# AdamBeedell/MLX8-WS-Audio-Transformer

Hardware: AMD Instinct MI355X
Metric: 4s@16kHz clips/sec through mel+Whisper-small encoder (higher is better)
Workload: dtype fp16; 1 GPU; int16 PCM [B,64000] in HBM -> Whisper log-mel [B,80,3000] -> Whisper-small encoder -> hidden [B,1500,768] fp32; mode=parity (clip zero-padded to 30 s, as the reference computes), precision=f16f8, fp16_exact_projection_matrices=0 of 48 (found by the library at upload), parallelism=dp1 (clip shards, no data-path collective)

## Files before the change

mlx8-ws-audio-transformer_amd/csrc/attention_f8.hip:

```cpp
#include <type_traits>
#include "common.h"

extern int g_attn_shape;

namespace {

typedef int i32x4_t __attribute__((ext_vector_type(4)));

constexpr int KB = 64;
constexpr int PL16 = KB * 64 * 2;
constexpr int PL8 = KB * 64;
constexpr int STAGE = 2 * PL16 + 4 * PL8;
constexpr int OFF_K16 = 0, OFF_V16 = PL16, OFF_K8 = 2 * PL16, OFF_KL8 = 2 * PL16 + PL8, OFF_V8 = 2 * PL16 + 2 * PL8, OFF_VL8 = 2 * PL16 + 3 * PL8;

struct Attn8Args {
  const bf16_t *q16, *k16, *v16;
  const uint8_t *q8, *ql8, *k8, *kl8, *v8, *vl8;
  bf16_t* o16; uint8_t *o8, *ol8; float* o_f32;
  float* lse;
  int B, H, S;
  char* o_ilv;
};

__device__ __forceinline__ int swz16(int row) { return (row >> 1) & 7; }
__device__ __forceinline__ int swz_v16(int row) { return ((row >> 1) & 1) << 2; }
__device__ __forceinline__ int swz_k8(int row) { return (row >> 2) & 3; }
__device__ __forceinline__ int swz_v8(int row) { return ((row >> 3) & 1) << 1; }

template <int E>
__device__ __forceinline__ int fp8x4_scaled(float a, float b, float c, float d) {
  typedef short s16x2 __attribute__((ext_vector_type(2)));
  constexpr float inv = pow2f(-E);
  s16x2 r = {0, 0};
  r = __builtin_amdgcn_cvt_scalef32_pk_fp8_f32(r, a, b, inv, false);
  r = __builtin_amdgcn_cvt_scalef32_pk_fp8_f32(r, c, d, inv, true);
  return __builtin_bit_cast(int, r);
}

constexpr int K3_SLOT = PL16 + 2 * PL8, V3_SLOT = PL16, K3_O8 = PL16, K3_OL8 = PL16 + PL8, V3_BASE = 3 * K3_SLOT, RING3_BYTES = 3 * (K3_SLOT + V3_SLOT);
template <int NW>
struct KvLaneOff {
  unsigned o16[8 / NW];
  unsigned o16v[8 / NW];
  unsigned o8k, o8v;
};
template <int NW>
__device__ __forceinline__ KvLaneOff<NW> kv_lane_off(int last, int wave, int lane) {
  KvLaneOff<NW> o;
#pragma unroll
  for (int i = 0; i < 8 / NW; ++i) {
    const int p = (i * NW + wave) * 64 + lane, row = p >> 3;
    o.o16[i] = (unsigned)(min(row, last) * 64 + (((p & 7) ^ swz16(row)) << 3)) * 2u;
    o.o16v[i] = (unsigned)(min(row, last) * 64 + (((p & 7) ^ swz_v16(row)) << 3)) * 2u;
  }
  const int p = (wave & 3) * 64 + lane, row = p >> 2;
  o.o8k = (unsigned)(min(row, last) * 64 + (((p & 3) ^ swz_k8(row)) << 4));
  o.o8v = (unsigned)(min(row, last) * 64 + (((p & 3) ^ swz_v8(row)) << 4));
  return o;
}
template <int NW, bool ISK, bool W8 = true, bool RING3 = false>
__device__ __forceinline__ void stage_kv1(const Attn8Args& a, int64_t head_off, int kt, unsigned stage, int wave, const KvLaneOff<NW>& lo) {
  const int64_t tile_off = head_off + (int64_t)kt * (KB * 64);
  const bf16_t* p16 = (ISK ? a.k16 : a.v16) + tile_off;
  const uint8_t* p8 = (ISK ? a.k8 : a.v8) + tile_off;
  const uint8_t* pl8 = (ISK ? a.kl8 : a.vl8) + tile_off;
  constexpr int O16 = RING3 ? 0 : (ISK ? OFF_K16 : OFF_V16), O8 = RING3 ? K3_O8 : (ISK ? OFF_K8 : OFF_V8), OL8 = RING3 ? K3_OL8 : (ISK ? OFF_KL8 : OFF_VL8);
#pragma unroll
  for (int i = 0; i < 8 / NW; ++i) glds16_asm_sbase(p16, ISK ? lo.o16[i] : lo.o16v[i], stage + O16 + (i * NW + wave) * 1024);
  if constexpr (!W8) return;
  const int grp = wave & 3;
  const unsigned off = ISK ? lo.o8k : lo.o8v;
  if (NW == 4) {
    glds16_asm_sbase(p8, off, stage + O8 + grp * 1024);
    glds16_asm_sbase(pl8, off, stage + OL8 + grp * 1024);
  } else {
    glds16_asm_sbase(wave < 4 ? p8 : pl8, off, stage + (wave < 4 ? O8 : OL8) + grp * 1024);
  }
}

template <int NW, bool PV8>
__global__ __launch_bounds__(64 * NW, 2) void attention_f16f8_pipe_kernel(Attn8Args a) {
  constexpr int QB = 32 * NW;
  extern __shared__ __attribute__((aligned(16))) char smem[];
  const int lane = threadIdx.x & 63;
  const int wave = __builtin_amdgcn_readfirstlane(threadIdx.x >> 6);
  const int nqb = (a.S + QB - 1) / QB;
  const int nwg = nqb * a.B * a.H;
  const int logical = xcd_contiguous(blockIdx.x, nwg);
  const int bh = logical / nqb;
  const int b = bh / a.H, h = bh - b * a.H;
  const int q0 = (logical - bh * nqb) * QB + wave * 32;
  const int64_t head_off = (int64_t)bh * a.S * 64;
  const int ql = lane & 31, half = lane >> 5;

  bf16x8 q16[4];
  i32x8 q8, ql8;
  {
    int q = q0 + ql; q = q < a.S ? q : a.S - 1;
    const int64_t off = head_off + (int64_t)q * 64;
#pragma unroll
    for (int ks = 0; ks < 4; ++ks) q16[ks] = *reinterpret_cast<const bf16x8*>(a.q16 + off + half * 8 + ks * 16);
    const uint4 x0 = *reinterpret_cast<const uint4*>(a.q8 + off + half * 32), x1 = *reinterpret_cast<const uint4*>(a.q8 + off + half * 32 + 16);
    const uint4 y0 = *reinterpret_cast<const uint4*>(a.ql8 + off + half * 32), y1 = *reinterpret_cast<const uint4*>(a.ql8 + off + half * 32 + 16);
    q8 = (i32x8){(int)x0.x, (int)x0.y, (int)x0.z, (int)x0.w, (int)x1.x, (int)x1.y, (int)x1.z, (int)x1.w};
    ql8 = (i32x8){(int)y0.x, (int)y0.y, (int)y0.z, (int)y0.w, (int)y1.x, (int)y1.y, (int)y1.z, (int)y1.w};
  }
  f32x16 oacc[2] = {(f32x16){}, (f32x16){}};
  float m_run = -1.0e30f, l_run = 0.f;

  int koff[4], k8off[2];
#pragma unroll
  for (int ks = 0; ks < 4; ++ks) koff[ks] = ql * 128 + (((2 * ks + half) ^ swz16(ql)) << 4);
#pragma unroll
  for (int c = 0; c < 2; ++c) k8off[c] = ql * 64 + (((2 * half + c) ^ swz_k8(ql)) << 4);
  const int g = lane >> 4, li = lane & 15, qq = li >> 2, pp = li & 3;
  const int vkey = 4 * (g >> 1) + qq;
  const int voff = vkey * 128 + (((2 * (g & 1) + (pp >> 1)) ^ swz_v16(vkey)) << 4) + 8 * (pp & 1);
  const int voffx = voff ^ 64;
  const int tq = li >> 1, tp = li & 1;
  const int v8key = 8 * (tq >> 2) + (tq & 3) + 4 * (g >> 1);
  const int v8off = v8key * 64 + ((((g & 1)) ^ swz_v8(v8key)) << 4) + 8 * tp;

  const int ntiles = (a.S + KB - 1) / KB;

  constexpr int NSLOT = PV8 ? 24 : 20, DEPTH = 2, RING = DEPTH + 1;
  constexpr bool RING3 = !PV8;
  static_assert(!RING3 || NW == 4, "the ring form runs on four waves (its counted vmcnt waits assume one group of each e4m3 plane per wave)");
  constexpr int KO8 = RING3 ? K3_O8 : OFF_K8, KOL8 = RING3 ? K3_OL8 : OFF_KL8, VO16 = RING3 ? 0 : OFF_V16;
  const unsigned lds0 = (unsigned)(uintptr_t)(__attribute__((address_space(3))) const char*)(smem);
  auto kslot = [&](int t) -> unsigned { return RING3 ? lds0 + (t % 3) * K3_SLOT : lds0 + (t & 1) * STAGE; };
  auto vslot = [&](int t) -> unsigned { return RING3 ? lds0 + V3_BASE + (t % 3) * V3_SLOT : lds0 + (t & 1) * STAGE; };
  struct RdAddr { unsigned k16[4], k8[2], v0, v1, v8[2]; };
  auto rd_addr = [&](unsigned kb, unsigned vb) {
    RdAddr r;
    constexpr bool PIN = !PV8;
#pragma unroll
    for (int ks = 0; ks < 4; ++ks) { r.k16[ks] = kb + koff[ks]; if constexpr (PIN) asm volatile("" : "+v"(r.k16[ks])); }
#pragma unroll
    for (int c = 0; c < 2; ++c) { r.k8[c] = kb + k8off[c]; if constexpr (PIN) asm volatile("" : "+v"(r.k8[c])); }
    r.v0 = vb + VO16 + voff; r.v1 = vb + VO16 + voffx;
    if constexpr (PIN) asm volatile("" : "+v"(r.v0), "+v"(r.v1));
    if constexpr (PV8) { r.v8[0] = vb + v8off; r.v8[1] = vb + (v8off ^ 32); }
    else r.v8[0] = r.v8[1] = 0;
    return r;
  };
  auto lds128 = [](unsigned addr) { return *(const __attribute__((address_space(3))) i32x4_t*)(uintptr_t)addr; };
  auto read_slot = [&](auto slot_t, const RdAddr& ra, i32x8& f) {
    constexpr int SLOT = decltype(slot_t)::value;
    if constexpr (SLOT < 12) {
      constexpr int kt2 = SLOT / 6, w = SLOT % 6;
      if constexpr (w < 2) {
        constexpr int pl = (w == 0 ? KO8 : KOL8) + kt2 * 2048;
        const i32x4_t x0 = lds128(ra.k8[0] + pl), x1 = lds128(ra.k8[1] + pl);
        f = (i32x8){x0[0], x0[1], x0[2], x0[3], x1[0], x1[1], x1[2], x1[3]};
      } else {
        const i32x4_t x0 = lds128(ra.k16[w - 2] + kt2 * 4096);
        f[0] = x0[0]; f[1] = x0[1]; f[2] = x0[2]; f[3] = x0[3];
      }
    } else if constexpr (SLOT < 20) {
      constexpr int I = SLOT - 12, kt2 = I >> 2, s2 = (I >> 1) & 1, et = I & 1;
      constexpr int cst = kt2 * 4096 + s2 * 2048;
      const unsigned a0 = (et == 0 ? ra.v0 : ra.v1) + cst, a1 = a0 + 1024;
      const i32x2 va = __builtin_bit_cast(i32x2, __builtin_amdgcn_ds_read_tr16_b64_v4i16((__attribute__((address_space(3))) bf16x4*)(uintptr_t)a0));
      const i32x2 vb2 = __builtin_bit_cast(i32x2, __builtin_amdgcn_ds_read_tr16_b64_v4i16((__attribute__((address_space(3))) bf16x4*)(uintptr_t)a1));
      f[0] = va[0]; f[1] = va[1]; f[2] = vb2[0]; f[3] = vb2[1];
    } else {
      constexpr int I = SLOT - 20, et = I >> 1, lo = I & 1;
#pragma unroll
      for (int n = 0; n < 4; ++n) {
        const i32x2 x = __builtin_amdgcn_ds_read_tr8_b64_v2i32((__attribute__((address_space(3))) i32x2*)(uintptr_t)(ra.v8[et] + (lo ? OFF_VL8 : OFF_V8) + n * 1024));
        f[2 * n] = x[0]; f[2 * n + 1] = x[1];
      }
    }
  };
  const KvLaneOff<NW> lo_full = kv_lane_off<NW>(KB - 1, wave, lane);
  auto lane_off = [&](int t) -> KvLaneOff<NW> {
    if ((a.S % KB) != 0 && t == ntiles - 1) return kv_lane_off<NW>(a.S - 1 - t * KB, wave, lane);
    return lo_full;
  };

  stage_kv1<NW, true, true, RING3>(a, head_off, 0, kslot(0), wave, lane_off(0));
  stage_kv1<NW, false, PV8, RING3>(a, head_off, 0, vslot(0), wave, lane_off(0));
  if (ntiles > 1) stage_kv1<NW, true, true, RING3>(a, head_off, 1, kslot(1), wave, lane_off(1));
  if constexpr (RING3) {
    if (ntiles > 1) stage_kv1<NW, false, PV8, RING3>(a, head_off, 1, vslot(1), wave, lane_off(1));
    if (ntiles > 2) stage_kv1<NW, true, true, RING3>(a, head_off, 2, kslot(2), wave, lane_off(2));
  }
  asm volatile("s_waitcnt vmcnt(0)" ::: "memory");
  __syncthreads();
  f32x16 sa[2], sb[2];
  auto qk_mma = [&](auto slot_t, const i32x8& f, f32x16 (&sn)[2]) {
    constexpr int SLOT = decltype(slot_t)::value, kt2 = SLOT / 6, w = SLOT % 6;
    if constexpr (w == 0) sn[kt2] = mfma32_f8<e8m0(-kF8KV), e8m0(-kF8Q - kF8Lo)>(f, ql8, (f32x16){});
    else if constexpr (w == 1) sn[kt2] = mfma32_f8<e8m0(-kF8KV - kF8Lo), e8m0(-kF8Q)>(f, q8, sn[kt2]);
    else {
      const bf16x8 kh = __builtin_bit_cast(bf16x8, (i32x4_t){f[0], f[1], f[2], f[3]});
      sn[kt2] = mfma32<true>(kh, q16[w - 2], sn[kt2]);
    }
  };
  {
    i32x8 ring[RING];
    const RdAddr ra0 = rd_addr(kslot(0), vslot(0));
    [&]<int... P>(std::integer_sequence<int, P...>) { (read_slot(std::integral_constant<int, P>{}, ra0, ring[P]), ...); }(std::make_integer_sequence<int, DEPTH>{});
    [&]<int... I>(std::integer_sequence<int, I...>) {
      ([&] {
        if constexpr (I + DEPTH < 12) read_slot(std::integral_constant<int, I + DEPTH>{}, ra0, ring[(I + DEPTH) % RING]);
        qk_mma(std::integral_constant<int, I>{}, ring[I % RING], sa);
      }(), ...);
    }(std::make_integer_sequence<int, 12>{});
  }
  asm volatile("s_waitcnt lgkmcnt(0)" ::: "memory");
  __syncthreads();

  auto iter = [&](auto last_t, auto tail_t, int kt, f32x16 (&sc)[2], f32x16 (&sn)[2]) {
    constexpr bool LAST = decltype(last_t)::value, TAIL = decltype(tail_t)::value;
    constexpr int FIRST = LAST ? 12 : 0;
    const RdAddr ra = rd_addr(kslot(kt + 1), vslot(kt));
    if constexpr (!LAST) {
      if constexpr (RING3) {
        if (kt + 3 < ntiles) stage_kv1<NW, true, true, true>(a, head_off, kt + 3, kslot(kt), wave, lane_off(kt + 3));
        if (kt + 2 < ntiles) stage_kv1<NW, false, false, true>(a, head_off, kt + 2, vslot(kt + 2), wave, lane_off(kt + 2));
      } else {
        if (kt + 2 < ntiles) stage_kv1<NW, true>(a, head_off, kt + 2, kslot(kt), wave, lane_off(kt + 2));
        stage_kv1<NW, false, PV8>(a, head_off, kt + 1, vslot(kt + 1), wave, lane_off(kt + 1));
      }
    }
    bf16x8 p16[4];
    i32x8 p8, pl8;
    float tmax = -1.0e30f, m_new, alpha, psum = 0.f;
    auto valu_chunk = [&](auto c_t) {
      constexpr int C = decltype(c_t)::value;
      if constexpr (C < 2) {
#pragma unroll
        for (int r = 0; r < 16; ++r) {
          if (TAIL) {
            const int key = kt * KB + C * 32 + (r & 3) + 8 * (r >> 2) + 4 * half;
            sc[C][r] = key < a.S ? sc[C][r] : -1.0e30f;
          }
          tmax = fmaxf(tmax, sc[C][r]);
        }
        if constexpr (C == 1) {
          tmax = fmaxf(tmax, __shfl_xor(tmax, 32));
          m_new = fmaxf(m_run, tmax);
          alpha = __builtin_amdgcn_exp2f(m_run - m_new);
          m_run = m_new;
        }
      } else if constexpr (C < 10) {
        constexpr int e = C - 2, kt2 = e >> 2, r4 = e & 3;
#pragma unroll
        for (int j = 0; j < 4; ++j) {
          const float pv = __builtin_amdgcn_exp2f(sc[kt2][4 * r4 + j] - m_new);
          sc[kt2][4 * r4 + j] = pv;
          psum += pv;
          p16[2 * kt2 + (r4 >> 1)][4 * (r4 & 1) + j] = (short)f32_to_f16(pv);
        }
      } else if constexpr (C < 12) {
        constexpr int et = C - 10;
#pragma unroll
        for (int r = 0; r < 16; ++r) {
          oacc[et][r] *= alpha;
        }
        if constexpr (et == 1) l_run = l_run * alpha + psum;
      } else if constexpr (C < 20 && PV8) {
        constexpr int I = C - 12, c2 = I >> 2, r4 = I & 3;
        float lo[4];
#pragma unroll
        for (int j = 0; j < 4; ++j) lo[j] = __builtin_fmaf(f16_to_f32((bf16_t)p16[2 * c2 + (r4 >> 1)][4 * (r4 & 1) + j]), -1.0f, sc[c2][4 * r4 + j]);
        p8[4 * c2 + r4] = fp8x4_scaled<kF8P>(sc[c2][4 * r4], sc[c2][4 * r4 + 1], sc[c2][4 * r4 + 2], sc[c2][4 * r4 + 3]);
        pl8[4 * c2 + r4] = fp8x4_scaled<kF8P + kF8Lo>(lo[0], lo[1], lo[2], lo[3]);
      }
    };
    auto mma = [&](auto slot_t, const i32x8& f) {
      constexpr int SLOT = decltype(slot_t)::value;
      if constexpr (SLOT < 12) qk_mma(slot_t, f, sn);
      else if constexpr (SLOT < 20) {
        constexpr int I = SLOT - 12, kt2 = I >> 2, s2 = (I >> 1) & 1, et = I & 1;
        const bf16x8 vh = __builtin_bit_cast(bf16x8, (i32x4_t){f[0], f[1], f[2], f[3]});
        oacc[et] = mfma32<true>(vh, p16[2 * kt2 + s2], oacc[et]);
      } else {
        constexpr int I = SLOT - 20, et = I >> 1, lo = I & 1;
        if constexpr (lo == 0) oacc[et] = mfma32_f8<e8m0(-kF8KV), e8m0(-kF8P - kF8Lo)>(f, pl8, oacc[et]);
        else oacc[et] = mfma32_f8<e8m0(-kF8KV - kF8Lo), e8m0(-kF8P)>(f, p8, oacc[et]);
      }
    };
    i32x8 ring[RING];
    [&]<int... P>(std::integer_sequence<int, P...>) { (read_slot(std::integral_constant<int, FIRST + P>{}, ra, ring[(FIRST + P) % RING]), ...); }(std::make_integer_sequence<int, DEPTH>{});
    if constexpr (LAST) {
      [&]<int... C>(std::integer_sequence<int, C...>) { (valu_chunk(std::integral_constant<int, C>{}), ...); }(std::make_integer_sequence<int, 12>{});
    }
    [&]<int... J>(std::integer_sequence<int, J...>) {
      ([&] {
        constexpr int I = FIRST + J;
        if constexpr (I + DEPTH < NSLOT) read_slot(std::integral_constant<int, I + DEPTH>{}, ra, ring[(I + DEPTH) % RING]);
        if constexpr (!LAST || I >= 12) valu_chunk(std::integral_constant<int, I>{});
        __builtin_amdgcn_sched_barrier(0);
        mma(std::integral_constant<int, I>{}, ring[I % RING]);
        __builtin_amdgcn_sched_barrier(0);
      }(), ...);
    }(std::make_integer_sequence<int, NSLOT - FIRST>{});
    if constexpr (RING3 && !LAST) {
      constexpr int NK = 8 / NW + 2, NV = 8 / NW;
      if (kt + 3 < ntiles) asm volatile("s_waitcnt vmcnt(%0)" ::"n"(NK + NV) : "memory");
      else if (kt + 2 < ntiles) asm volatile("s_waitcnt vmcnt(%0)" ::"n"(NV) : "memory");
      else asm volatile("s_waitcnt vmcnt(0)" ::: "memory");
    } else {
      asm volatile("s_waitcnt vmcnt(0)" ::: "memory");
    }
    __syncthreads();
  };
  int kt = 0;
  for (; kt + 2 < ntiles; kt += 2) {
    iter(std::false_type{}, std::false_type{}, kt, sa, sb);
    iter(std::false_type{}, std::false_type{}, kt + 1, sb, sa);
  }
  if (kt + 2 == ntiles) {
    iter(std::false_type{}, std::false_type{}, kt, sa, sb);
    if (a.S % KB) iter(std::true_type{}, std::true_type{}, kt + 1, sb, sa);
    else iter(std::true_type{}, std::false_type{}, kt + 1, sb, sa);
  } else {
    if (a.S % KB) iter(std::true_type{}, std::true_type{}, kt, sa, sb);
    else iter(std::true_type{}, std::false_type{}, kt, sa, sb);
  }

  const float l_tot = l_run + __shfl_xor(l_run, 32);
  const float inv = 1.0f / l_tot;
  const int q = q0 + ql;
  if (a.lse && q < a.S && half == 0) a.lse[(int64_t)bh * a.S + q] = m_run + __builtin_amdgcn_logf(l_tot);
  if (q < a.S) {
    const int64_t row = ((int64_t)b * a.S + q) * (a.H * 64) + h * 64;
#pragma unroll
    for (int et = 0; et < 2; ++et)
#pragma unroll
      for (int g4 = 0; g4 < 4; ++g4) {
        const int e = 32 * et + 8 * g4 + 4 * half;
        float v[4];
#pragma unroll
        for (int j = 0; j < 4; ++j) v[j] = oacc[et][4 * g4 + j] * inv;
        if (a.o_f32) {
          *reinterpret_cast<float4*>(a.o_f32 + row + e) = make_float4(v[0], v[1], v[2], v[3]);
        } else {
          uint2 h16; unsigned hi8, lo8;
          f16f8x4<kF8Act>(v, h16, hi8, lo8);
          if (a.o_ilv) { store_ilv4(a.o_ilv, row + e, h16, hi8, lo8); continue; }
          *reinterpret_cast<uint2*>(a.o16 + row + e) = h16;
          if (a.o8) *reinterpret_cast<unsigned*>(a.o8 + row + e) = hi8;
          *reinterpret_cast<unsigned*>(a.ol8 + row + e) = lo8;
        }
      }
  }
}

template <int NW, bool PV8>
int launch_pipe(const Attn8Args& a, hipStream_t s) {
  constexpr int lds = PV8 ? 2 * STAGE : RING3_BYTES;
  constexpr int QB = 32 * NW;
  return launch_kernel<attention_f16f8_pipe_kernel<NW, PV8>>(dim3(((a.S + QB - 1) / QB) * a.B * a.H), dim3(64 * NW), lds, s, a);
}

struct F8Form { int nw; bool pv8; };
F8Form f16f8_form(bool with_lse, int B, int H, int S) {
  if (g_attn_shape == 4) return {4, true};
  if (g_attn_shape == 5) return {8, true};
  if (g_attn_shape == 6) return {4, false};
  if (with_lse) return {(int64_t)((S + 255) / 256) * B * H >= 256 ? 8 : 4, true};
  return {4, false};
}

}

int g_attn_shape = 0;
void awt_attn_force_shape(int v) { g_attn_shape = v; }

bool attention_f16f8_reads_v8(bool with_lse) { return with_lse || f16f8_form(with_lse, 1, 1, 1).pv8; }

int launch_attention_f16f8(awt_ctx* c, const F8Planes& q, const F8Planes& k, const F8Planes& v, const F8Planes& o, float* o_f32,
                           float* lse, int B, int H, int S, hipStream_t s, char* o_ilv) {
  AWT_REQUIRE(B > 0 && H > 0 && S > 0, AWT_ERR_INVALID, "attention: bad shape");
  AWT_REQUIRE(q.p16 && q.hi8 && q.lo8 && k.p16 && k.hi8 && k.lo8 && v.p16 && v.hi8 && v.lo8, AWT_ERR_INVALID, "attention (f16f8): null plane");
  AWT_REQUIRE(o_f32 || o_ilv || (o.p16 && o.lo8), AWT_ERR_INVALID, "attention (f16f8): null output plane (hi8 may be null: not consumed)");
  AWT_REQUIRE(!o_ilv || (H * 64) % 64 == 0, AWT_ERR_INVALID, "attention (f16f8): split-line output needs whole 64-element line pairs per row");
  Attn8Args a{q.p16, k.p16, v.p16, q.hi8, q.lo8, k.hi8, k.lo8, v.hi8, v.lo8, o.p16, o.hi8, o.lo8, o_f32, lse, B, H, S};
  a.o_ilv = o_f32 ? nullptr : o_ilv;
  ProfScope prof(c, AWT_PROF_ATTENTION, s, 4.0 * (double)B * H * (double)S * S * 64);
  const F8Form f = f16f8_form(lse != nullptr, B, H, S);
  if (f.pv8) return f.nw == 8 ? launch_pipe<8, true>(a, s) : launch_pipe<4, true>(a, s);
  return launch_pipe<4, false>(a, s);
}
```

Before: 1418 clips/s.

## Restructure ring-3 attention loop with compile-time slot phases and software-pipelined softmax max

For the 3-slot ring path, the main KV loop is unrolled by six so each iteration's LDS slot offsets become compile-time constants folded into immediate addresses, and staging runs without tail checks. The next tile's row max and rescale factor are now computed at the end of the current iteration, overlapping with its MMAs, rather than at the start of the next. Exponentials are packed to fp16 in pairs, and the accumulator rescale is interleaved with the exp chunks. The goal is fewer address computations, fewer branches and better VALU/MFMA overlap, at the cost of larger code and more register pressure.

```diff
diff --git a/mlx8-ws-audio-transformer_amd/csrc/attention_f8.hip b/mlx8-ws-audio-transformer_amd/csrc/attention_f8.hip
--- a/mlx8-ws-audio-transformer_amd/csrc/attention_f8.hip
+++ b/mlx8-ws-audio-transformer_amd/csrc/attention_f8.hip
@@ -6,6 +6,8 @@
 namespace {
 
 typedef int i32x4_t __attribute__((ext_vector_type(4)));
+typedef float f32x2 __attribute__((ext_vector_type(2)));
+typedef _Float16 f16x2 __attribute__((ext_vector_type(2)));
 
 constexpr int KB = 64;
 constexpr int PL16 = KB * 64 * 2;
@@ -144,22 +146,23 @@
     else r.v8[0] = r.v8[1] = 0;
     return r;
   };
+  using I0 = std::integral_constant<int, 0>;
   auto lds128 = [](unsigned addr) { return *(const __attribute__((address_space(3))) i32x4_t*)(uintptr_t)addr; };
-  auto read_slot = [&](auto slot_t, const RdAddr& ra, i32x8& f) {
-    constexpr int SLOT = decltype(slot_t)::value;
+  auto read_slot = [&](auto slot_t, const RdAddr& ra, i32x8& f, auto kadd_t, auto vadd_t) {
+    constexpr int SLOT = decltype(slot_t)::value, KADD = decltype(kadd_t)::value, VADD = decltype(vadd_t)::value;
     if constexpr (SLOT < 12) {
       constexpr int kt2 = SLOT / 6, w = SLOT % 6;
       if constexpr (w < 2) {
-        constexpr int pl = (w == 0 ? KO8 : KOL8) + kt2 * 2048;
+        constexpr int pl = (w == 0 ? KO8 : KOL8) + kt2 * 2048 + KADD;
         const i32x4_t x0 = lds128(ra.k8[0] + pl), x1 = lds128(ra.k8[1] + pl);
         f = (i32x8){x0[0], x0[1], x0[2], x0[3], x1[0], x1[1], x1[2], x1[3]};
       } else {
-        const i32x4_t x0 = lds128(ra.k16[w - 2] + kt2 * 4096);
+        const i32x4_t x0 = lds128(ra.k16[w - 2] + kt2 * 4096 + KADD);
         f[0] = x0[0]; f[1] = x0[1]; f[2] = x0[2]; f[3] = x0[3];
       }
     } else if constexpr (SLOT < 20) {
       constexpr int I = SLOT - 12, kt2 = I >> 2, s2 = (I >> 1) & 1, et = I & 1;
-      constexpr int cst = kt2 * 4096 + s2 * 2048;
+      constexpr int cst = kt2 * 4096 + s2 * 2048 + VADD;
       const unsigned a0 = (et == 0 ? ra.v0 : ra.v1) + cst, a1 = a0 + 1024;
       const i32x2 va = __builtin_bit_cast(i32x2, __builtin_amdgcn_ds_read_tr16_b64_v4i16((__attribute__((address_space(3))) bf16x4*)(uintptr_t)a0));
       const i32x2 vb2 = __builtin_bit_cast(i32x2, __builtin_amdgcn_ds_read_tr16_b64_v4i16((__attribute__((address_space(3))) bf16x4*)(uintptr_t)a1));
@@ -201,10 +204,10 @@
   {
     i32x8 ring[RING];
     const RdAddr ra0 = rd_addr(kslot(0), vslot(0));
-    [&]<int... P>(std::integer_sequence<int, P...>) { (read_slot(std::integral_constant<int, P>{}, ra0, ring[P]), ...); }(std::make_integer_sequence<int, DEPTH>{});
+    [&]<int... P>(std::integer_sequence<int, P...>) { (read_slot(std::integral_constant<int, P>{}, ra0, ring[P], I0{}, I0{}), ...); }(std::make_integer_sequence<int, DEPTH>{});
     [&]<int... I>(std::integer_sequence<int, I...>) {
       ([&] {
-        if constexpr (I + DEPTH < 12) read_slot(std::integral_constant<int, I + DEPTH>{}, ra0, ring[(I + DEPTH) % RING]);
+        if constexpr (I + DEPTH < 12) read_slot(std::integral_constant<int, I + DEPTH>{}, ra0, ring[(I + DEPTH) % RING], I0{}, I0{});
         qk_mma(std::integral_constant<int, I>{}, ring[I % RING], sa);
       }(), ...);
     }(std::make_integer_sequence<int, 12>{});
@@ -212,114 +215,244 @@
   asm volatile("s_waitcnt lgkmcnt(0)" ::: "memory");
   __syncthreads();
 
-  auto iter = [&](auto last_t, auto tail_t, int kt, f32x16 (&sc)[2], f32x16 (&sn)[2]) {
-    constexpr bool LAST = decltype(last_t)::value, TAIL = decltype(tail_t)::value;
-    constexpr int FIRST = LAST ? 12 : 0;
-    const RdAddr ra = rd_addr(kslot(kt + 1), vslot(kt));
-    if constexpr (!LAST) {
-      if constexpr (RING3) {
+  if constexpr (RING3) {
+    float alpha, tmax, tmax_x;
+    auto max_sub = [&](auto c_t, auto tail_t, int t, f32x16 (&s)[2]) {
+      constexpr int C = decltype(c_t)::value;
+      constexpr bool TAIL = decltype(tail_t)::value;
+      if constexpr (C == 0) tmax = -1.0e30f;
+#pragma unroll
+      for (int r = 0; r < 16; ++r) {
+        if (TAIL) {
+          const int key = t * KB + C * 32 + (r & 3) + 8 * (r >> 2) + 4 * half;
+          s[C][r] = key < a.S ? s[C][r] : -1.0e30f;
+        }
+        tmax = fmaxf(tmax, s[C][r]);
+      }
+      if constexpr (C == 1) tmax_x = __shfl_xor(tmax, 32);
+    };
+    auto max_fin = [&] {
+      tmax = fmaxf(tmax, tmax_x);
+      const float m_new = fmaxf(m_run, tmax);
+      alpha = __builtin_amdgcn_exp2f(m_run - m_new);
+      m_run = m_new;
+      asm volatile("" : "+v"(alpha), "+v"(m_run));
+    };
+    max_sub(std::integral_constant<int, 0>{}, std::true_type{}, 0, sa);
+    max_sub(std::integral_constant<int, 1>{}, std::true_type{}, 0, sa);
+    max_fin();
+
+    const RdAddr rb = rd_addr(lds0, lds0 + V3_BASE);
+    auto iter = [&](auto last_t, auto ntail_t, auto ph_t, int kt, f32x16 (&sc)[2], f32x16 (&sn)[2]) {
+      constexpr bool LAST = decltype(last_t)::value;
+      constexpr int PH = decltype(ph_t)::value;
+      constexpr int FIRST = LAST ? 12 : 0;
+      using KAdd = std::integral_constant<int, PH < 0 ? 0 : ((PH + 1) % 3) * K3_SLOT>;
+      using VAdd = std::integral_constant<int, PH < 0 ? 0 : PH * V3_SLOT>;
+      RdAddr ra;
+      if constexpr (PH < 0) ra = rd_addr(kslot(kt + 1), vslot(kt));
+      else ra = rb;
+      if constexpr (PH >= 0) {
+        static_assert(!LAST);
+        stage_kv1<NW, true, true, true>(a, head_off, kt + 3, lds0 + PH * K3_SLOT, wave, lo_full);
+        stage_kv1<NW, false, false, true>(a, head_off, kt + 2, lds0 + V3_BASE + ((PH + 2) % 3) * V3_SLOT, wave, lo_full);
+      } else if constexpr (!LAST) {
         if (kt + 3 < ntiles) stage_kv1<NW, true, true, true>(a, head_off, kt + 3, kslot(kt), wave, lane_off(kt + 3));
         if (kt + 2 < ntiles) stage_kv1<NW, false, false, true>(a, head_off, kt + 2, vslot(kt + 2), wave, lane_off(kt + 2));
-      } else {
+      }
+      unsigned p16[4][4];
+      float psum = 0.f;
+      auto exps = [&](auto e_t, auto j0_t, auto n_t) {
+        constexpr int E = decltype(e_t)::value, J0 = decltype(j0_t)::value, N = decltype(n_t)::value, kt2 = E >> 2, r4 = E & 3;
+#pragma unroll
+        for (int j = J0; j < J0 + N; j += 2) {
+          const float pv0 = __builtin_amdgcn_exp2f(sc[kt2][4 * r4 + j] - m_run), pv1 = __builtin_amdgcn_exp2f(sc[kt2][4 * r4 + j + 1] - m_run);
+          psum += pv0;
+          psum += pv1;
+          unsigned w = __builtin_bit_cast(unsigned, __builtin_convertvector((f32x2){pv0, pv1}, f16x2));
+          asm volatile("" : "+v"(w));
+          p16[2 * kt2 + (r4 >> 1)][2 * (r4 & 1) + j / 2] = w;
+        }
+        asm volatile("" : "+v"(psum));
+      };
+      auto valu_chunk = [&](auto g_t) {
+        constexpr int G = decltype(g_t)::value;
+        using I4 = std::integral_constant<int, 4>;
+        using I2 = std::integral_constant<int, 2>;
+        if constexpr (G == 1 || G == 2) exps(std::integral_constant<int, G - 1>{}, I0{}, I4{});
+        else if constexpr (G >= 3 && G <= 6) {
+          constexpr int et = (G - 3) >> 1, r0 = 8 * ((G - 3) & 1);
+#pragma unroll
+          for (int r = r0; r < r0 + 8; ++r) {
+            float x = oacc[et][r] * alpha;
+            asm volatile("" : "+v"(x));
+            oacc[et][r] = x;
+          }
+        } else if constexpr (G == 7 || G == 8) exps(std::integral_constant<int, G - 5>{}, I0{}, I4{});
+        else if constexpr (G >= 9 && G <= 16) {
+          exps(std::integral_constant<int, 4 + (G - 9) / 2>{}, std::integral_constant<int, 2 * ((G - 9) & 1)>{}, I2{});
+          if constexpr (G == 16) { l_run = __builtin_fmaf(l_run, alpha, psum); asm volatile("" : "+v"(l_run)); }
+        } else if constexpr (G >= 17 && !LAST) {
+          if constexpr (G < 19) max_sub(std::integral_constant<int, G - 17>{}, ntail_t, kt + 1, sn);
+          else max_fin();
+        }
+      };
+      auto mma = [&](auto slot_t, const i32x8& f) {
+        constexpr int SLOT = decltype(slot_t)::value;
+        if constexpr (SLOT < 12) qk_mma(slot_t, f, sn);
+        else {
+          constexpr int I = SLOT - 12, kt2 = I >> 2, s2 = (I >> 1) & 1, et = I & 1;
+          const bf16x8 vh = __builtin_bit_cast(bf16x8, (i32x4_t){f[0], f[1], f[2], f[3]});
+          const unsigned(&pw)[4] = p16[2 * kt2 + s2];
+          oacc[et] = mfma32<true>(vh, __builtin_bit_cast(bf16x8, (i32x4_t){(int)pw[0], (int)pw[1], (int)pw[2], (int)pw[3]}), oacc[et]);
+        }
+      };
+      i32x8 ring[RING];
+      [&]<int... P>(std::integer_sequence<int, P...>) { (read_slot(std::integral_constant<int, FIRST + P>{}, ra, ring[(FIRST + P) % RING], KAdd{}, VAdd{}), ...); }(std::make_integer_sequence<int, DEPTH>{});
+      if constexpr (LAST) {
+        [&]<int... C>(std::integer_sequence<int, C...>) { (valu_chunk(std::integral_constant<int, C + 1>{}), ...); }(std::make_integer_sequence<int, 12>{});
+      }
+      [&]<int... J>(std::integer_sequence<int, J...>) {
+        ([&] {
+          constexpr int I = FIRST + J;
+          if constexpr (I + DEPTH < NSLOT) read_slot(std::integral_constant<int, I + DEPTH>{}, ra, ring[(I + DEPTH) % RING], KAdd{}, VAdd{});
+          if constexpr (!LAST || I > 12) valu_chunk(std::integral_constant<int, I>{});
+          __builtin_amdgcn_sched_barrier(0);
+          mma(std::integral_constant<int, I>{}, ring[I % RING]);
+          __builtin_amdgcn_sched_barrier(0);
+        }(), ...);
+      }(std::make_integer_sequence<int, NSLOT - FIRST>{});
+      if constexpr (!LAST) {
+        constexpr int NK = 8 / NW + 2, NV = 8 / NW;
+        if (PH >= 0 || kt + 3 < ntiles) asm volatile("s_waitcnt vmcnt(%0)" ::"n"(NK + NV) : "memory");
+        else if (kt + 2 < ntiles) asm volatile("s_waitcnt vmcnt(%0)" ::"n"(NV) : "memory");
+        else asm volatile("s_waitcnt vmcnt(0)" ::: "memory");
+        __syncthreads();
+      }
+    };
+    using Ph = std::integral_constant<int, -1>;
+    int kt = 0;
+    for (; kt + 9 < ntiles; kt += 6) {
+      iter(std::false_type{}, std::false_type{}, std::integral_constant<int, 0>{}, kt, sa, sb);
+      iter(std::false_type{}, std::false_type{}, std::integral_constant<int, 1>{}, kt + 1, sb, sa);
+      iter(std::false_type{}, std::false_type{}, std::integral_constant<int, 2>{}, kt + 2, sa, sb);
+      iter(std::false_type{}, std::false_type{}, std::integral_constant<int, 0>{}, kt + 3, sb, sa);
+      iter(std::false_type{}, std::false_type{}, std::integral_constant<int, 1>{}, kt + 4, sa, sb);
+      iter(std::false_type{}, std::false_type{}, std::integral_constant<int, 2>{}, kt + 5, sb, sa);
+    }
+    for (; kt + 3 < ntiles; kt += 2) {
+      iter(std::false_type{}, std::false_type{}, Ph{}, kt, sa, sb);
+      iter(std::false_type{}, std::false_type{}, Ph{}, kt + 1, sb, sa);
+    }
+    if (kt + 3 == ntiles) {
+      iter(std::false_type{}, std::false_type{}, Ph{}, kt, sa, sb);
+      iter(std::false_type{}, std::true_type{}, Ph{}, kt + 1, sb, sa);
+      iter(std::true_type{}, std::false_type{}, Ph{}, kt + 2, sa, sb);
+    } else if (kt + 2 == ntiles) {
+      iter(std::false_type{}, std::true_type{}, Ph{}, kt, sa, sb);
+      iter(std::true_type{}, std::false_type{}, Ph{}, kt + 1, sb, sa);
+    } else {
+      iter(std::true_type{}, std::false_type{}, Ph{}, kt, sa, sb);
+    }
+  } else {
+    auto iter = [&](auto last_t, auto tail_t, int kt, f32x16 (&sc)[2], f32x16 (&sn)[2]) {
+      constexpr bool LAST = decltype(last_t)::value, TAIL = decltype(tail_t)::value;
+      constexpr int FIRST = LAST ? 12 : 0;
+      const RdAddr ra = rd_addr(kslot(kt + 1), vslot(kt));
+      if constexpr (!LAST) {
         if (kt + 2 < ntiles) stage_kv1<NW, true>(a, head_off, kt + 2, kslot(kt), wave, lane_off(kt + 2));
         stage_kv1<NW, false, PV8>(a, head_off, kt + 1, vslot(kt + 1), wave, lane_off(kt + 1));
       }
-    }
-    bf16x8 p16[4];
-    i32x8 p8, pl8;
-    float tmax = -1.0e30f, m_new, alpha, psum = 0.f;
-    auto valu_chunk = [&](auto c_t) {
-      constexpr int C = decltype(c_t)::value;
-      if constexpr (C < 2) {
-#pragma unroll
-        for (int r = 0; r < 16; ++r) {
-          if (TAIL) {
-            const int key = kt * KB + C * 32 + (r & 3) + 8 * (r >> 2) + 4 * half;
-            sc[C][r] = key < a.S ? sc[C][r] : -1.0e30f;
+      bf16x8 p16[4];
+      i32x8 p8, pl8;
+      float tmax = -1.0e30f, m_new, alpha, psum = 0.f;
+      auto valu_chunk = [&](auto c_t) {
+        constexpr int C = decltype(c_t)::value;
+        if constexpr (C < 2) {
+#pragma unroll
+          for (int r = 0; r < 16; ++r) {
+            if (TAIL) {
+              const int key = kt * KB + C * 32 + (r & 3) + 8 * (r >> 2) + 4 * half;
+              sc[C][r] = key < a.S ? sc[C][r] : -1.0e30f;
+            }
+            tmax = fmaxf(tmax, sc[C][r]);
           }
-          tmax = fmaxf(tmax, sc[C][r]);
-        }
-        if constexpr (C == 1) {
-          tmax = fmaxf(tmax, __shfl_xor(tmax, 32));
-          m_new = fmaxf(m_run, tmax);
-          alpha = __builtin_amdgcn_exp2f(m_run - m_new);
-          m_run = m_new;
-        }
-      } else if constexpr (C < 10) {
-        constexpr int e = C - 2, kt2 = e >> 2, r4 = e & 3;
-#pragma unroll
-        for (int j = 0; j < 4; ++j) {
-          const float pv = __builtin_amdgcn_exp2f(sc[kt2][4 * r4 + j] - m_new);
-          sc[kt2][4 * r4 + j] = pv;
-          psum += pv;
-          p16[2 * kt2 + (r4 >> 1)][4 * (r4 & 1) + j] = (short)f32_to_f16(pv);
-        }
-      } else if constexpr (C < 12) {
-        constexpr int et = C - 10;
-#pragma unroll
-        for (int r = 0; r < 16; ++r) {
-          oacc[et][r] *= alpha;
-        }
-        if constexpr (et == 1) l_run = l_run * alpha + psum;
-      } else if constexpr (C < 20 && PV8) {
-        constexpr int I = C - 12, c2 = I >> 2, r4 = I & 3;
-        float lo[4];
-#pragma unroll
-        for (int j = 0; j < 4; ++j) lo[j] = __builtin_fmaf(f16_to_f32((bf16_t)p16[2 * c2 + (r4 >> 1)][4 * (r4 & 1) + j]), -1.0f, sc[c2][4 * r4 + j]);
-        p8[4 * c2 + r4] = fp8x4_scaled<kF8P>(sc[c2][4 * r4], sc[c2][4 * r4 + 1], sc[c2][4 * r4 + 2], sc[c2][4 * r4 + 3]);
-        pl8[4 * c2 + r4] = fp8x4_scaled<kF8P + kF8Lo>(lo[0], lo[1], lo[2], lo[3]);
-      }
+          if constexpr (C == 1) {
+            tmax = fmaxf(tmax, __shfl_xor(tmax, 32));
+            m_new = fmaxf(m_run, tmax);
+            alpha = __builtin_amdgcn_exp2f(m_run - m_new);
+            m_run = m_new;
+          }
+        } else if constexpr (C < 10) {
+          constexpr int e = C - 2, kt2 = e >> 2, r4 = e & 3;
+#pragma unroll
+          for (int j = 0; j < 4; ++j) {
+            const float pv = __builtin_amdgcn_exp2f(sc[kt2][4 * r4 + j] - m_new);
+            sc[kt2][4 * r4 + j] = pv;
+            psum += pv;
+            p16[2 * kt2 + (r4 >> 1)][4 * (r4 & 1) + j] = (short)f32_to_f16(pv);
+          }
+        } else if constexpr (C < 12) {
+          constexpr int et = C - 10;
+#pragma unroll
+          for (int r = 0; r < 16; ++r) {
+            oacc[et][r] *= alpha;
+          }
+          if constexpr (et == 1) l_run = l_run * alpha + psum;
+        } else if constexpr (C < 20 && PV8) {
+          constexpr int I = C - 12, c2 = I >> 2, r4 = I & 3;
+          float lo[4];
+#pragma unroll
+          for (int j = 0; j < 4; ++j) lo[j] = __builtin_fmaf(f16_to_f32((bf16_t)p16[2 * c2 + (r4 >> 1)][4 * (r4 & 1) + j]), -1.0f, sc[c2][4 * r4 + j]);
+          p8[4 * c2 + r4] = fp8x4_scaled<kF8P>(sc[c2][4 * r4], sc[c2][4 * r4 + 1], sc[c2][4 * r4 + 2], sc[c2][4 * r4 + 3]);
+          pl8[4 * c2 + r4] = fp8x4_scaled<kF8P + kF8Lo>(lo[0], lo[1], lo[2], lo[3]);
+        }
+      };
+      auto mma = [&](auto slot_t, const i32x8& f) {
+        constexpr int SLOT = decltype(slot_t)::value;
+        if constexpr (SLOT < 12) qk_mma(slot_t, f, sn);
+        else if constexpr (SLOT < 20) {
+          constexpr int I = SLOT - 12, kt2 = I >> 2, s2 = (I >> 1) & 1, et = I & 1;
+          const bf16x8 vh = __builtin_bit_cast(bf16x8, (i32x4_t){f[0], f[1], f[2], f[3]});
+          oacc[et] = mfma32<true>(vh, p16[2 * kt2 + s2], oacc[et]);
+        } else {
+          constexpr int I = SLOT - 20, et = I >> 1, lo = I & 1;
+          if constexpr (lo == 0) oacc[et] = mfma32_f8<e8m0(-kF8KV), e8m0(-kF8P - kF8Lo)>(f, pl8, oacc[et]);
+          else oacc[et] = mfma32_f8<e8m0(-kF8KV - kF8Lo), e8m0(-kF8P)>(f, p8, oacc[et]);
+        }
+      };
+      i32x8 ring[RING];
+      [&]<int... P>(std::integer_sequence<int, P...>) { (read_slot(std::integral_constant<int, FIRST + P>{}, ra, ring[(FIRST + P) % RING], I0{}, I0{}), ...); }(std::make_integer_sequence<int, DEPTH>{});
+      if constexpr (LAST) {
+        [&]<int... C>(std::integer_sequence<int, C...>) { (valu_chunk(std::integral_constant<int, C>{}), ...); }(std::make_integer_sequence<int, 12>{});
+      }
+      [&]<int... J>(std::integer_sequence<int, J...>) {
+        ([&] {
+          constexpr int I = FIRST + J;
+          if constexpr (I + DEPTH < NSLOT) read_slot(std::integral_constant<int, I + DEPTH>{}, ra, ring[(I + DEPTH) % RING], I0{}, I0{});
+          if constexpr (!LAST || I >= 12) valu_chunk(std::integral_constant<int, I>{});
+          __builtin_amdgcn_sched_barrier(0);
+          mma(std::integral_constant<int, I>{}, ring[I % RING]);
+          __builtin_amdgcn_sched_barrier(0);
+        }(), ...);
+      }(std::make_integer_sequence<int, NSLOT - FIRST>{});
+      asm volatile("s_waitcnt vmcnt(0)" ::: "memory");
+      __syncthreads();
     };
-    auto mma = [&](auto slot_t, const i32x8& f) {
-      constexpr int SLOT = decltype(slot_t)::value;
-      if constexpr (SLOT < 12) qk_mma(slot_t, f, sn);
-      else if constexpr (SLOT < 20) {
-        constexpr int I = SLOT - 12, kt2 = I >> 2, s2 = (I >> 1) & 1, et = I & 1;
-        const bf16x8 vh = __builtin_bit_cast(bf16x8, (i32x4_t){f[0], f[1], f[2], f[3]});
-        oacc[et] = mfma32<true>(vh, p16[2 * kt2 + s2], oacc[et]);
-      } else {
-        constexpr int I = SLOT - 20, et = I >> 1, lo = I & 1;
-        if constexpr (lo == 0) oacc[et] = mfma32_f8<e8m0(-kF8KV), e8m0(-kF8P - kF8Lo)>(f, pl8, oacc[et]);
-        else oacc[et] = mfma32_f8<e8m0(-kF8KV - kF8Lo), e8m0(-kF8P)>(f, p8, oacc[et]);
-      }
-    };
-    i32x8 ring[RING];
-    [&]<int... P>(std::integer_sequence<int, P...>) { (read_slot(std::integral_constant<int, FIRST + P>{}, ra, ring[(FIRST + P) % RING]), ...); }(std::make_integer_sequence<int, DEPTH>{});
-    if constexpr (LAST) {
-      [&]<int... C>(std::integer_sequence<int, C...>) { (valu_chunk(std::integral_constant<int, C>{}), ...); }(std::make_integer_sequence<int, 12>{});
-    }
-    [&]<int... J>(std::integer_sequence<int, J...>) {
-      ([&] {
-        constexpr int I = FIRST + J;
-        if constexpr (I + DEPTH < NSLOT) read_slot(std::integral_constant<int, I + DEPTH>{}, ra, ring[(I + DEPTH) % RING]);
-        if constexpr (!LAST || I >= 12) valu_chunk(std::integral_constant<int, I>{});
-        __builtin_amdgcn_sched_barrier(0);
-        mma(std::integral_constant<int, I>{}, ring[I % RING]);
-        __builtin_amdgcn_sched_barrier(0);
-      }(), ...);
-    }(std::make_integer_sequence<int, NSLOT - FIRST>{});
-    if constexpr (RING3 && !LAST) {
-      constexpr int NK = 8 / NW + 2, NV = 8 / NW;
-      if (kt + 3 < ntiles) asm volatile("s_waitcnt vmcnt(%0)" ::"n"(NK + NV) : "memory");
-      else if (kt + 2 < ntiles) asm volatile("s_waitcnt vmcnt(%0)" ::"n"(NV) : "memory");
-      else asm volatile("s_waitcnt vmcnt(0)" ::: "memory");
+    int kt = 0;
+    for (; kt + 2 < ntiles; kt += 2) {
+      iter(std::false_type{}, std::false_type{}, kt, sa, sb);
+      iter(std::false_type{}, std::false_type{}, kt + 1, sb, sa);
+    }
+    if (kt + 2 == ntiles) {
+      iter(std::false_type{}, std::false_type{}, kt, sa, sb);
+      if (a.S % KB) iter(std::true_type{}, std::true_type{}, kt + 1, sb, sa);
+      else iter(std::true_type{}, std::false_type{}, kt + 1, sb, sa);
     } else {
-      asm volatile("s_waitcnt vmcnt(0)" ::: "memory");
-    }
-    __syncthreads();
-  };
-  int kt = 0;
-  for (; kt + 2 < ntiles; kt += 2) {
-    iter(std::false_type{}, std::false_type{}, kt, sa, sb);
-    iter(std::false_type{}, std::false_type{}, kt + 1, sb, sa);
-  }
-  if (kt + 2 == ntiles) {
-    iter(std::false_type{}, std::false_type{}, kt, sa, sb);
-    if (a.S % KB) iter(std::true_type{}, std::true_type{}, kt + 1, sb, sa);
-    else iter(std::true_type{}, std::false_type{}, kt + 1, sb, sa);
-  } else {
-    if (a.S % KB) iter(std::true_type{}, std::true_type{}, kt, sa, sb);
-    else iter(std::true_type{}, std::false_type{}, kt, sa, sb);
+      if (a.S % KB) iter(std::true_type{}, std::true_type{}, kt, sa, sb);
+      else iter(std::true_type{}, std::false_type{}, kt, sa, sb);
+    }
+
   }
 
   const float l_tot = l_run + __shfl_xor(l_run, 32);
```

Measured after the change: 1449 clips/s (median of 6 runs). 2.2% higher.
